# WE-Autopilot/red_gym

Hardware: AMD Instinct MI355X
Metric: env steps/sec (all envs), 1080-beam lidar (higher is better)
Workload: dtype f64; 1 GPU; 65536 envs x 1 agent(s) per GPU, example_map, 1080 beams, RK4 single-track, noise+iTTC, lap logic, autoreset; random actions; envs_per_gpu=65536, agents=1, num_beams=1080, map=example_map

## Files before the change

### include/f110_hip.h

```cpp
#ifndef F110_HIP_H
#define F110_HIP_H

#include <stdint.h>

#ifdef __cplusplus
extern "C" {
#endif

#define F110_OK 0
#define F110_E_INVALID (-1)
#define F110_E_HIP (-2)
#define F110_E_NOMAP (-3)
#define F110_E_INDEX (-4)
#define F110_E_UNBOUND (-5)

#define F110_MAX_CARS (1 << 26)
#define F110_MAX_AGENTS 32
#define F110_MAX_MAPS 4096
#define F110_MAX_NOISE_SLOTS 64
#define F110_NOISE_INITIAL_ROWS 1024
#define F110_NUM_PARAMS 18
#define F110_RK4 1
#define F110_EULER 2

// ... 86 lines not shown
int f110_noise_set_floor(f110_handle *h, int64_t lo, void *stream);
int f110_noise_info(f110_handle *h, int64_t *lo, int64_t *hi, int64_t *cap, int32_t *slots, int64_t *bytes);
int f110_noise_read(f110_handle *h, int32_t slot, int64_t row0, int64_t n_rows, double *out_host);

#define F110_DEVERR_NOISE_WINDOW 0x1u
#define F110_DEVERR_BOUNDS 0x2u
#define F110_DEVERR_QP_LIMIT 0x4u
int f110_device_errors(f110_handle *h, uint32_t *flags_out);

int f110_bind(f110_handle *h, const f110_buffers *bufs);

int f110_reset(f110_handle *h, const double *poses_dev, const uint8_t *mask_dev, void *stream);

int f110_step(f110_handle *h, const double *actions_dev, void *stream);

int64_t f110_pack_env_size(f110_handle *h);
int f110_pack_env(f110_handle *h, int32_t env, double *out_dev, void *stream);

int f110_set_scan_stages(f110_handle *h, const char *spec);

int f110_set_scan_order(f110_handle *h, const int32_t *order_dev);
int f110_launch_epoch(f110_handle *h, int64_t *epoch);

#define F110_GRAPH_NODES 0
#define F110_GRAPH_CAPTURE 1
typedef struct f110_graph f110_graph;
int f110_graph_create(f110_handle *h, const double *actions_dev, int32_t how, f110_graph **out);
int f110_graph_launch(f110_graph *g, void *stream);
int f110_graph_info(f110_graph *g, int32_t *nodes, const char *dot_path);
void f110_graph_destroy(f110_graph *g);

int f110_profile_begin(f110_handle *h, int32_t max_launches);
int f110_profile_every(f110_handle *h, int32_t every);
int f110_profile_end(f110_handle *h, double *scan_ms_total, int32_t *launches);

int f110_pure_pursuit_prepare(f110_handle *h, const double *waypoints, int32_t M, double cell, double margin, void *stream);
int f110_pure_pursuit(f110_handle *h, const double *waypoints, int32_t M, double lookahead, double vgain,
                      double wheelbase, double max_reacquire, const double *state, int32_t n,
                      double *actions, void *stream);

int64_t f110_pure_pursuit_workspace(int32_t total_points, int32_t K);
int f110_pure_pursuit_tracks(f110_handle *h, const double *waypoints, const int32_t *offsets_dev,
                             const int32_t *offsets_host, int32_t K, const int32_t *track_of_car, double lookahead,
                             double vgain, double wheelbase, double max_reacquire, const double *state, int32_t n,
                             double *actions, double *workspace, int32_t boxes_valid, void *stream);

// ... 363 lines not shown
```

### red_gym_amd/_lib.py

```python
import ctypes as C
import os

_HERE = os.path.dirname(os.path.abspath(__file__))
LIB_PATH = os.environ.get('F110_LIB') or os.path.join(_HERE, 'libf110_hip.so')

F110_MAX_AGENTS = 32
F110_MAX_NOISE_SLOTS = 64
F110_MAX_MAPS = 4096
F110_NUM_PARAMS = 18
F110_RK4, F110_EULER = 1, 2
E_INVALID, E_HIP, E_NOMAP, E_INDEX, E_UNBOUND = -1, -2, -3, -4, -5

PARAM_KEYS = ['mu', 'C_Sf', 'C_Sr', 'lf', 'lr', 'h', 'm', 'I', 's_min', 's_max', 'sv_min', 'sv_max',
              'v_switch', 'a_max', 'v_min', 'v_max', 'width', 'length']


class Config(C.Structure):
    _fields_ = [('num_envs', C.c_int32), ('num_agents', C.c_int32), ('num_beams', C.c_int32),
                ('theta_dis', C.c_int32), ('integrator', C.c_int32), ('ego_idx', C.c_int32),
                ('device', C.c_int32), ('autoreset', C.c_int32), ('fov', C.c_double), ('eps', C.c_double),
                ('max_range', C.c_double), ('timestep', C.c_double), ('ttc_thresh', C.c_double),
                ('params', C.c_double * F110_NUM_PARAMS)]


# ... 196 lines not shown
    'f110_set_params_slots': [_VP, _VP, _I32],
    'f110_set_params_slot': [_VP, _I32, _VP, _I32],
    'f110_assign_params': [_VP, _VP],
    'f110_set_side_distance_slots': [_VP, _VP, _I32],
    'f110_set_noise_table': [_VP, _VP, _I64],
    'f110_set_noise_slot': [_VP, _I32, _VP, _I64],
    'f110_set_noise_generator': [_VP, _I32, _VP, _D],
    'f110_assign_noise': [_VP, _VP],
    'f110_set_noise_per_env': [_VP, _VP, _D],
    'f110_noise_ensure': [_VP, _I64, _VP],
    'f110_noise_prefetch': [_VP, _I64],
    'f110_noise_set_floor': [_VP, _I64, _VP],
    'f110_noise_info': [_VP, C.POINTER(C.c_int64), C.POINTER(C.c_int64), C.POINTER(C.c_int64), C.POINTER(C.c_int32), C.POINTER(C.c_int64)],
    'f110_noise_read': [_VP, _I32, _I64, _I64, _VP],
    'f110_device_errors': [_VP, C.POINTER(C.c_uint32)],
    'f110_bind': [_VP, C.POINTER(Buffers)],
    'f110_reset': [_VP, _VP, _VP, _VP],
    'f110_step': [_VP, _VP, _VP],
    'f110_pack_env_size': [_VP],
    'f110_pack_env': [_VP, _I32, _VP, _VP],
    'f110_set_scan_stages': [_VP, C.c_char_p],
    'f110_launch_epoch': [_VP, C.POINTER(C.c_int64)],
    'f110_set_scan_order': [_VP, _VP],
    'f110_graph_create': [_VP, _VP, _I32, C.POINTER(_VP)],
    'f110_graph_launch': [_VP, _VP],
    'f110_graph_info': [_VP, C.POINTER(C.c_int32), C.c_char_p],
    'f110_graph_destroy': [_VP],
    'f110_pure_pursuit': [_VP, _VP, _I32, _D, _D, _D, _D, _VP, _I32, _VP, _VP],
    'f110_pure_pursuit_prepare': [_VP, _VP, _I32, _D, _D, _VP],
    'f110_pure_pursuit_workspace': [_I32, _I32],
    'f110_pure_pursuit_tracks': [_VP, _VP, _VP, _VP, _I32, _VP, _D, _D, _D, _D, _VP, _I32, _VP, _VP, _I32, _VP],
    'f110_progress_validate': [_VP, _VP, _I32, _VP, _VP, _VP, _VP, _VP, _I32],
    'f110_progress_install': [_VP, _VP, _VP, _I32, _VP, _VP, _VP, _VP, _VP, _I32],
    'f110_progress_bind': [_VP, C.POINTER(ProgressBuffers)],
    'f110_progress_update': [_VP, _VP],
    'f110_shaping_validate': [C.POINTER(ShapingConfig), _I32],
    'f110_shaping_install': [_VP, C.POINTER(ShapingConfig)],
    'f110_shaping_bind': [_VP, C.POINTER(ShapingBuffers)],
    'f110_shaping_update': [_VP, _VP],
    'f110_shaping_terms': [C.POINTER(ShapingConfig), _VP, _VP, _VP, _I32, _VP, _VP, _VP, _VP, _VP, _VP],
    'f110_shaping_terms_bits': [C.POINTER(ShapingConfig), _VP, _VP, _VP, _I32, _VP, _VP, _VP, _VP, _VP, _VP],
    'f110_pathfollow_validate': [C.POINTER(PathFollowConfig), _I32],
    'f110_pathfollow_install': [_VP, C.POINTER(PathFollowConfig)],
    'f110_pathfollow_bind': [_VP, C.POINTER(PathFollowBuffers)],
    'f110_pathfollow_act': [_VP, _VP, _VP, _VP],
    'f110_pathfollow_update': [_VP, _VP],
# ... 135 lines not shown
```

### red_gym_amd/csrc/f110_handle.h

```cpp
#pragma once
#include "f110_common.h"
#include "f110_device.h"
#include "f110_map.h"
#include "f110_noise.h"
#include "f110_plangrid.h"
#include "f110_scan_plan.h"

namespace f110 { struct OppPair; }

struct PlanGridDev {
    PlanGrid g;
    DevBuf<uint8_t> d_count; DevBuf<uint16_t> d_cand;
    hipError_t upload(const PlanGrid &geometry, const std::vector<uint8_t> &count, const std::vector<uint16_t> &cand)
    {
        hipError_t e = d_count.upload(count.data(), count.size());
        if (e == hipSuccess) e = d_cand.upload(cand.data(), cand.size());
        g = geometry; g.count = d_count.get(); g.cand = d_cand.get();
        return e;
    }
};

struct NoiseRows {
    const double *base;
    int cap, mask, slots;
// ... 83 lines not shown
    struct Replay {
        bool on = false, bound = false;
        f110_replay_config cfg;
        int rows = 0, cols = 0;
        f110_replay_buffers bufs;
    } replay;
    struct Episodes {
        bool on = false, bound = false;
        f110_episodes_config cfg;
        f110_episodes_buffers bufs;
    } episodes;
    const int32_t *scan_order = nullptr;
    DevBuf<uint32_t> d_err;
    std::vector<double> h_side;
    DevBuf<double> d_side_slots;
    int side_n_slots = 0;
    std::vector<double> h_side_slot0;
    double side_slots_max = 0.0;
    struct MapSlot {
        DevBuf<uint16_t> d_cells, d_cells_far;
        DevBuf<double> d_lut, d_lut_lds, d_dt;
        MapDev dev;
        bool used = false, ident = false, pow2 = false;
    };
    MapSlot slots[F110_MAX_MAPS];
    DevBuf<MapDev> d_maps;
    DevBuf<int32_t> d_env_map;
    std::vector<int32_t> h_env_map;
    bool multi = false;
    bool wg_single = false;
    bool ident = false, pow2 = false;
    double theta_inc = 0;
    std::vector<Event> prof_ev;
    int prof_n = 0, prof_every = 1, prof_seq = 0;
    bool prof_on = false;
};

int check_device(const f110_handle *h, const char *who);
int noise_init(f110_handle *h);
int alloc_opp_pairs(f110_handle *h);
```

### red_gym_amd/csrc/f110_map.h

```cpp
#pragma once
#include <hip/hip_runtime.h>
#include <stddef.h>
#include <stdint.h>

#pragma clang fp contract(off)

namespace f110 {

constexpr int LUT_LDS = 1024;
constexpr unsigned SLOT_OOB = 0, SLOT_FAR = LUT_LDS - 1;
constexpr unsigned LDS_RANKS = LUT_LDS - 2;
constexpr unsigned OFF_FAR = 8 * SLOT_FAR;
constexpr unsigned CODE_ESC = 65535;
__host__ __device__ inline unsigned cell_code(unsigned rank) { return rank < LDS_RANKS ? 8u * (rank + 1u) : OFF_FAR; }
__host__ __device__ inline int map_rows_padded(int H) { return ((H + 2 + 7) >> 3) << 3; }
__host__ __device__ inline size_t map_cells(int H, int W) { return (size_t)((W >> 3) + 2) * map_rows_padded(H) * 8; }
__host__ __device__ inline size_t cell_elem(int r, int c, int Hp) { return ((size_t)((c >> 3) + 1) * Hp + (size_t)(r + 1)) * 8 + (size_t)(c & 7); }

struct MapDev {
    const uint16_t *cells;
    const uint16_t *cells_far;
    unsigned cells_bytes;
    unsigned strip_bytes;
    const double *lut;
    const double *lut_lds;
    const double *dt;
    int H, W;
    double res, rinv, ox, oy, oc, os, wres, hres, oob;
    unsigned lut_len;
};

}
```

### red_gym_amd/csrc/f110_mapgen.h

```cpp
#pragma once
#include "f110_map.h"

#pragma clang fp contract(off)

namespace f110 {

constexpr unsigned EDT_NONE = 0xffffffffu;

static __global__ __launch_bounds__(256) void edt_columns_kernel(const uint8_t *mask, int H, int W, unsigned *g)
{
    const int x = blockIdx.x * blockDim.x + threadIdx.x;
    if (x >= W) return;
    unsigned d = EDT_NONE;
    for (int y = 0; y < H; y++) {
        const size_t i = (size_t)y * W + x;
        d = mask[i] ? (d == EDT_NONE ? EDT_NONE : d + 1) : 0u;
        g[i] = d;
    }
    d = EDT_NONE;
    for (int y = H - 1; y >= 0; y--) {
        const size_t i = (size_t)y * W + x;
        d = mask[i] ? (d == EDT_NONE ? EDT_NONE : d + 1) : 0u;
        const unsigned up = g[i];
        g[i] = d < up ? d : up;
// ... 107 lines not shown
    return word_prefix[v >> 5] + __popc(bits[v >> 5] & ((1u << (v & 31)) - 1u));
}

static __global__ __launch_bounds__(256) void map_encode_kernel(const unsigned *d2, int H, int W, int Hp, const unsigned *bits,
                                                         const unsigned *word_prefix, double res, uint16_t *cells,
                                                         uint16_t *cells_far, double *dt)
{
    const size_t i = (size_t)blockIdx.x * blockDim.x + threadIdx.x;
    if (i >= (size_t)H * W) return;
    const unsigned v = d2[i];
    const unsigned rank = d2_rank(bits, word_prefix, v);
    const size_t t = cell_elem((int)(i / W), (int)(i % W), Hp);
    cells[t] = (uint16_t)cell_code(rank);
    cells_far[t] = (uint16_t)(rank < CODE_ESC ? rank : CODE_ESC);
    dt[i] = res * sqrt((double)v);
}

static __global__ __launch_bounds__(256) void map_fill_border_kernel(uint16_t *cells, uint16_t *cells_far, size_t n)
{
    const size_t i = (size_t)blockIdx.x * blockDim.x + threadIdx.x;
    if (i >= n) return;
    cells[i] = 0;
    cells_far[i] = 0;
}

static __global__ __launch_bounds__(256) void map_lut_kernel(const unsigned *bits, int n_words, const unsigned *word_prefix, double res,
                                                      double *lut, unsigned n_lut)
{
    const int w = blockIdx.x * blockDim.x + threadIdx.x;
    if (w >= n_words) return;
    unsigned b = bits[w], rank = word_prefix[w];
    while (b && rank < n_lut) {
        const int bit = __ffs(b) - 1;
        b &= b - 1;
        lut[rank++] = res * sqrt((double)((unsigned)w * 32u + (unsigned)bit));
    }
}


struct TrackSeg { double ax, ay, ex, ey, inv_l2; };
constexpr int TRACK_CHUNK = 256;

static __global__ __launch_bounds__(256) void track_mask_kernel(const double *pts, int n_pts, int closed, int H, int W, double x0,
                                                         double y0, double pixel, double offset, double half_stroke,
                                                         uint8_t *mask)
{
// ... 33 lines not shown
```

### red_gym_amd/csrc/f110_maps.hip

```cpp
#include "f110_handle.h"
#include "f110_mapgen.h"

static int commit_map(f110_handle *h, int slot, f110_handle::MapSlot &&ns, int H, int W, double res, double ox, double oy, double oc,
                      double os, double oob)
{
    MapDev &m = ns.dev;
    memset(&m, 0, sizeof(m));
    m.cells = ns.d_cells.get(); m.cells_far = ns.d_cells_far.get(); m.lut = ns.d_lut.get(); m.lut_lds = ns.d_lut_lds.get(); m.dt = ns.d_dt.get();
    m.H = H; m.W = W; m.strip_bytes = (unsigned)map_rows_padded(H) * 16u; m.cells_bytes = (unsigned)(ns.d_cells.size() * sizeof(uint16_t));
    m.res = res; m.rinv = 1.0 / res;
    m.ox = ox; m.oy = oy; m.oc = oc; m.os = os;
    m.wres = W * res;
    m.hres = H * res;
    m.oob = oob;
    m.lut_len = (unsigned)ns.d_lut.size();
    int e = 0;
    ns.pow2 = std::frexp(res, &e) == 0.5;
    ns.ident = (oc == 1.0 && os == 0.0);
    ns.used = true;
    if (!h->d_maps.get()) {
        DevBuf<MapDev> maps;
        HIP_TRY(maps.alloc(F110_MAX_MAPS));
        HIP_TRY(hipMemset(maps.get(), 0, sizeof(MapDev) * F110_MAX_MAPS));
        h->d_maps = std::move(maps);
    }
    HIP_TRY(hipMemcpy(h->d_maps.get() + slot, &m, sizeof(MapDev), hipMemcpyHostToDevice));
    h->slots[slot] = std::move(ns);
    h->ident = h->pow2 = true;
    for (const auto &u : h->slots)
        if (u.used) { h->ident = h->ident && u.ident; h->pow2 = h->pow2 && u.pow2; }
// ... 255 lines not shown
```

### red_gym_amd/csrc/f110_scan.h

```cpp
#pragma once
#include "f110_bounds.h"
#include "f110_device.h"
#include "f110_map.h"
#include "f110_scan_plan.h"

#pragma clang fp contract(off)

namespace f110 {

constexpr int REFILL_MIN_IDLE = 44;

typedef unsigned u32x4 __attribute__((ext_vector_type(4)));
struct MapView {
    __amdgpu_buffer_rsrc_t cells_rsrc;
    u32x4 cells_words;
    unsigned row_bias, strip_m16;
    const MapDev *desc;
    int H, W;
    double res, rinv, ox, oy, oc, os, wres, hres;
    double nox, noy;
    F110_BOUNDS_ONLY(uint32_t *err = nullptr; unsigned cells_bytes = 0;)
    __device__ void init(const MapDev &m)
    {
        F110_BOUNDS_ONLY(cells_bytes = m.cells_bytes;)
        cells_rsrc = __builtin_amdgcn_make_buffer_rsrc(const_cast<uint16_t *>(m.cells), 0, (int)m.cells_bytes, 0x00020000);
        cells_words.x = __builtin_amdgcn_readfirstlane((unsigned)(unsigned long long)m.cells);
        cells_words.y = __builtin_amdgcn_readfirstlane((unsigned)((unsigned long long)m.cells >> 32) & 0xffffu);
        cells_words.z = __builtin_amdgcn_readfirstlane(m.cells_bytes); cells_words.w = __builtin_amdgcn_readfirstlane(0x00020000u);
        row_bias = m.strip_bytes + 16u; strip_m16 = m.strip_bytes - 16u; desc = &m; H = m.H; W = m.W; res = m.res; rinv = m.rinv;
        ox = m.ox; oy = m.oy; oc = m.oc; os = m.os; wres = m.wres; hres = m.hres;
        nox = -m.ox * m.rinv; noy = -m.oy * m.rinv;
    }
};

struct ScanDev {
    int nb, theta_dis;
    double fov, eps, max_range, inc;
    unsigned long long inc_fx;
    int cs_len;
    const double2 *cs;
};

template <bool IDENT, bool POW2>
__device__ inline void cell_index(const MapView &m, double x, double y, int &ci, int &ri)
{
    double xr = 0, yr = 0, qx, qy;
    if (IDENT && POW2) {
        qx = __builtin_fma(x, m.rinv, m.nox);
        qy = __builtin_fma(y, m.rinv, m.noy);
    } else {
// ... 18 lines not shown
    }
}

__device__ inline unsigned cell_offset(const MapView &m, int ci, int ri)
{
    const int cc = med3_i32(ci, -1, m.W);
    const int rr = med3_i32(ri, -1, m.H);
    unsigned row16;
    asm("v_lshl_add_u32 %0, %1, 4, %2" : "=v"(row16) : "v"(rr), "s"(m.row_bias));
    unsigned rc;
    asm("v_lshl_add_u32 %0, %1, 1, %2" : "=v"(rc) : "v"(cc), "v"(row16));
    return (unsigned)(__mul24(cc >> 3, (int)m.strip_m16) + (int)rc);
}

template <bool IDENT, bool POW2>
__device__ inline double dist_lookup(const MapView &m, const double *lds_lut, double x, double y)
{
    int ci, ri;
    cell_index<IDENT, POW2>(m, x, y, ci, ri);
    const unsigned off = cell_offset(m, ci, ri);
    unsigned code = (unsigned)(unsigned short)__builtin_amdgcn_raw_buffer_load_b16(m.cells_rsrc, (int)off, 0, 0);
#if defined(F110_BOUNDS)
    F110_BCHK(off + 2u <= m.cells_bytes, BT_LUT_CODE, m.err);
    F110_BCHK(code <= OFF_FAR && (code & 7u) == 0u, BT_LUT_CODE, m.err);
    code = code <= OFF_FAR ? (code & ~7u) : 0u;
#endif
    double d = *reinterpret_cast<const double *>(reinterpret_cast<const char *>(lds_lut) + code);
    asm volatile("" : "+v"(d));
    return d;
}

template <bool IDENT, bool POW2>
__device__ inline double dist_lookup_far(const MapView &m, double x, double y)
{
    int ci, ri;
    cell_index<IDENT, POW2>(m, x, y, ci, ri);
    unsigned off = cell_offset(m, ci, ri);
    const MapDev *dp = m.desc;
    asm volatile("" : "+s"(dp));
#if defined(F110_BOUNDS)
    F110_BCHK(off + 2u <= dp->cells_bytes, BT_CELLS_FAR, m.err);
    if (off + 2u > dp->cells_bytes) off = 0u;
#endif
    unsigned rank = *reinterpret_cast<const uint16_t *>(reinterpret_cast<const char *>(dp->cells_far) + (size_t)off);
    const bool inside = (unsigned)ri < (unsigned)m.H && (unsigned)ci < (unsigned)m.W;
#if defined(F110_BOUNDS)
    F110_BCHK(rank == CODE_ESC || rank < dp->lut_len, BT_LUT_RANK, m.err);
    if (rank != CODE_ESC && rank >= dp->lut_len) rank = 0u;
// ... 219 lines not shown
    double ttc_thresh;
    uint8_t *in_collision;
    const uint8_t *pending_reset;
    int reset_only;
    const uint16_t *chunk_beam0;
    const int32_t *order;
    int wg_single;
    int n_maps;
    const double *side_slots;
    const int32_t *env_params;
    int side_n_slots;
    float *out_f32;
    double *out_f64;
    uint32_t *lookups;
};

static_assert(__is_trivially_copyable(ScanArgs), "ScanArgs is copied into the kernarg segment byte for byte");
static_assert(offsetof(ScanArgs, maps) == 0, "kernarg re-read assumes the argument block starts with ScanArgs");
static_assert(sizeof(((ScanArgs *)0)->stage_cars) == SCAN_MAX_STAGES * sizeof(int) &&
              sizeof(((ScanArgs *)0)->stage_log2w) == SCAN_MAX_STAGES * sizeof(int), "stage list capacity");
static_assert(sizeof(ScanArgs) <= 4096, "kernarg segment size");

constexpr int SCAN_MIN_WAVES = 8;
template <bool IDENT, bool POW2, int SM>
__global__ __launch_bounds__(SCAN_THREADS, SCAN_MIN_WAVES) void scan_kernel(ScanArgs a)
{
    constexpr bool STEP = SM >= 1;
    __shared__ struct __attribute__((aligned(16))) { double lut[LUT_LDS]; int chunk0[MAX_CHUNKS]; } s_mem;
    double *const s_lut = s_mem.lut;
    int *const s_chunk0 = s_mem.chunk0;
#if defined(__HIP_DEVICE_COMPILE__)
    const ScanArgs *rare = (const ScanArgs *)__builtin_amdgcn_kernarg_segment_ptr();
#else
    const ScanArgs *rare = &a;
#endif
    const int nb = a.scan.nb;
    const int wave = __builtin_amdgcn_readfirstlane(threadIdx.x >> 6), lane = threadIdx.x & 63;
    const int wg_single = rare->wg_single;
    const int wid = wg_single ? (int)blockIdx.x : (int)blockIdx.x * SCAN_WAVES + wave;
    int wpc, car, part, lg;
    {
        int t = wid, c = 0, st = 0;
        const int ns = rare->n_stages;
        for (; st < ns; st++) {
            const int cars_s = rare->stage_cars[st], w = cars_s << rare->stage_log2w[st];
            if (t < w) break;
            t -= w; c += cars_s;
        }
        lg = st < ns ? rare->stage_log2w[st] : 0;
        wpc = 1 << lg; car = st < ns ? c + (t >> lg) : a.n_cars; part = t & (wpc - 1);
    }
    int car_c = rare->car_base + min(car, a.n_cars - 1);
    if (rare->order) car_c = rare->order[car_c];
    const int env_c = a.agents == 1 ? car_c : car_c / a.agents;
    F110_BCHK(rare->n_stages >= 1 && rare->n_stages <= SCAN_MAX_STAGES, BT_STAGE_LIST, rare->dev_err);
    int map_slot = a.env_map ? a.env_map[env_c] : 0;
#if defined(F110_BOUNDS)
    F110_BCHK((unsigned)map_slot < (unsigned)rare->n_maps, BT_MAP_SLOT, rare->dev_err);
    if ((unsigned)map_slot >= (unsigned)rare->n_maps) map_slot = 0;
#endif
    const MapDev &md = a.maps[map_slot];
    {
        const double2 *src = reinterpret_cast<const double2 *>(md.lut_lds);
        double2 *dst = reinterpret_cast<double2 *>(s_lut);
        for (int i = threadIdx.x; i < LUT_LDS / 2; i += SCAN_THREADS) dst[i] = src[i];
        if (SCAN_WAVES > 1 && wg_single)
            for (int k = 1; k < SCAN_WAVES; k++)
                for (int i = threadIdx.x + k * WAVE; i < LUT_LDS / 2; i += SCAN_THREADS) dst[i] = src[i];
    }
    static_assert(MAX_CHUNKS <= WAVE, "one pass of one wave stages the chunk table");
    if ((int)threadIdx.x < ((nb + 63) >> 6)) s_chunk0[threadIdx.x] = a.chunk_beam0[threadIdx.x];
    __syncthreads();
    MapView mv;
    mv.init(md);
    F110_BOUNDS_ONLY(mv.err = rare->dev_err;)
    if (car >= a.n_cars) return;
    car = car_c;
    const int nch = (nb + 63) >> 6;
    const int my_chunks = nch > part ? (nch - part + wpc - 1) >> lg : 0;
    const int owns_last = my_chunks > 0 && ((nch - 1) & (wpc - 1)) == part;
    const int nbl = my_chunks * 64 - (owns_last ? nch * 64 - nb : 0);
    if (a.reset_only && !a.pending_reset[env_c]) return;

    const double px = a.pose_src[(size_t)car * a.pose_stride];
    const double py = a.pose_src[(size_t)car * a.pose_stride + 1];
    const double yaw = a.pose_src[(size_t)car * a.pose_stride + a.yaw_off];
    const double eps = a.scan.eps, max_range = a.scan.max_range;

    const double vel = STEP ? a.state[(size_t)car * 7 + 3] : 0.0;
    const bool do_ttc = STEP && vel != 0.0;
    const double cand = a.ttc_thresh * fabs(vel) * 1.000000001;
    const double side_pre = do_ttc ? (rare->side_max + cand) + 1e-9 * (fabs(rare->side_max) + cand) : -__builtin_inf();
    const double *__restrict__ ns = nullptr;
    if (STEP) {
        const int row = a.noise_step[car];
        int slot = a.env_noise ? a.env_noise[env_c] : 0;
#if defined(F110_BOUNDS)
// ... 189 lines not shown
```

### red_gym_amd/csrc/f110_scan_plan.h

```cpp
#pragma once
#include "../../include/f110_hip.h"

#include <algorithm>
#include <cstdlib>
#include <cstring>
#include <vector>

int fail(int code, const char *fmt, ...);

namespace f110 {

constexpr int WAVE = 64;
constexpr int SCAN_WAVES = 2;
constexpr int SCAN_THREADS = SCAN_WAVES * WAVE;
constexpr int SCAN_MAX_STAGES = 8, SCAN_MAX_LOG2W = 3;
constexpr int MAX_CHUNKS = 64;

struct StageSpec { int cars, lg; };

inline bool parse_stage_spec(const char *p, std::vector<StageSpec> &spec, const char **why)
{
    spec.clear();
    int stars = 0;
    if (!p || !*p) { *why = "empty"; return false; }
    for (;;) {
        int cars = -1, lg = 0;
// ... 25 lines not shown
    std::vector<StageSpec> spec = override_spec;
    if (spec.empty()) {
        int wpc = n_cars <= 1024 ? 8 : (n_cars <= 2048 ? 4 : 1);
        const int nch = (num_beams + 63) / 64;
        while (wpc > 1 && wpc > nch) wpc /= 2;
        if (wpc > 1 || nch < 8) return {{n_cars, wpc >= 8 ? 3 : wpc >= 4 ? 2 : wpc >= 2 ? 1 : 0}};
        const int tail = std::min(agents >= 2 ? 4096 : 2048, n_cars / 2);
        spec = {{-1, 0}, {tail, 2}};
    }
    int fixed = 0;
    for (StageSpec &x : spec) if (x.cars >= 0) { x.cars -= x.cars % SCAN_WAVES; fixed += x.cars; }
    if (fixed > n_cars) { spec = {{-1, 0}}; fixed = 0; }
    bool star = false;
    for (StageSpec &x : spec) if (x.cars < 0 && !star) { x.cars = n_cars - fixed; star = true; }
    if (!star) spec.push_back({n_cars - fixed, 0});
    std::vector<StageSpec> stv;
    for (const StageSpec &x : spec) if (x.cars > 0) stv.push_back(x);
    for (size_t i = 0; i + 1 < stv.size(); i++)
        if (stv[i].cars % SCAN_WAVES) return {{n_cars, 0}};
    if (stv.size() > (size_t)SCAN_MAX_STAGES) return {{n_cars, 0}};
    return stv;
}

struct ScanPlanIn {
    int n_cars, agents, num_beams;
    const std::vector<StageSpec> *stages;
    bool step;
    const char *stores;
    bool multi, wg_single;
    int kind;
};

struct ScanLaunch {
    int car_base, n_cars;
    int kind;
    int sm;
    int n_stages, stage_cars[SCAN_MAX_STAGES], stage_log2w[SCAN_MAX_STAGES];
    int grid, block;
    bool wg_single, order, events;
};

template <typename EnvKind>
int plan_scan(const ScanPlanIn &in, EnvKind env_kind, std::vector<ScanLaunch> &out)
{
    const bool split = in.multi && in.kind != 3;
    const int num_envs = in.n_cars / in.agents;
    out.clear();
    for (int e0 = 0, e1 = num_envs; e0 < num_envs; e0 = e1) {
        ScanLaunch l = {};
        l.kind = split ? env_kind(e0) : in.kind;
        if (split)
            for (e1 = e0 + 1; e1 < num_envs && env_kind(e1) == l.kind; e1++) {}
        l.car_base = e0 * in.agents; l.n_cars = (e1 - e0) * in.agents;
        l.wg_single = in.multi && in.wg_single; l.order = in.step && !in.multi; l.events = in.step && e0 == 0;
        const std::vector<StageSpec> stv = scan_stage_list(*in.stages, l.n_cars, in.agents, in.num_beams);
        if (stv.size() < 1 || stv.size() > (size_t)SCAN_MAX_STAGES) return fail(F110_E_INVALID, "scan launch: %d stages (1..%d)", (int)stv.size(), SCAN_MAX_STAGES);
        long long cars = 0, waves = 0;
        for (const StageSpec &x : stv) {
            if (x.cars < 0 || x.lg < 0 || x.lg > SCAN_MAX_LOG2W) return fail(F110_E_INVALID, "scan launch: stage (%d cars, 2^%d waves per car) out of range", x.cars, x.lg);
            if (in.multi && !l.wg_single && (l.car_base + cars) % SCAN_WAVES) return fail(F110_E_INVALID, "scan launch: a stage of two-wave workgroups on a map per env starts at car %lld", l.car_base + cars);
            l.stage_cars[l.n_stages] = x.cars; l.stage_log2w[l.n_stages++] = x.lg;
            cars += x.cars; waves += x.cars << x.lg;
        }
        if (cars != l.n_cars) return fail(F110_E_INVALID, "scan launch: the stages cover %lld cars, the launch has %d", cars, l.n_cars);
        const bool plain = in.stores ? strcmp(in.stores, "plain") == 0 : l.n_cars > 327680;
        l.sm = !in.step ? 0 : plain ? 2 : 1;
        l.grid = (int)(l.wg_single ? waves : (waves + SCAN_WAVES - 1) / SCAN_WAVES);
        l.block = l.wg_single ? WAVE : SCAN_THREADS;
        out.push_back(l);
    }
    return F110_OK;
}

}
```

### red_gym_amd/csrc/f110_step.hip

```cpp
#include "f110_handle.h"
#include "f110_scan.h"
#include "f110_env.h"
#include "f110_mirrors.h"
#include "f110_noise_kernels.h"

int alloc_opp_pairs(f110_handle *h)
{
    if (h->cfg.num_agents < 2) return F110_OK;
    const size_t n = (size_t)h->cfg.num_envs * h->cfg.num_agents * (h->cfg.num_agents - 1);
    DevBuf<OppPair> pairs;
    DevBuf<uint8_t> was_pending;
    HIP_TRY(pairs.alloc(n));
    HIP_TRY(hipMemset(pairs.get(), 0, n * sizeof(OppPair)));
    HIP_TRY(was_pending.alloc((size_t)h->cfg.num_envs));
    HIP_TRY(hipMemset(was_pending.get(), 0, (size_t)h->cfg.num_envs));
    h->d_opp_pairs = std::move(pairs);
    h->d_was_pending = std::move(was_pending);
    return F110_OK;
}

struct KernelLaunch {
    const void *func;
    dim3 grid, block;
    unsigned shmem;
// ... 30 lines not shown
    memset(&s, 0, sizeof(s));
    ScanDev &d = s.scan;
    d.nb = h->cfg.num_beams; d.theta_dis = h->cfg.theta_dis; d.fov = h->cfg.fov; d.eps = h->cfg.eps;
    d.max_range = h->cfg.max_range; d.inc = h->theta_inc; d.inc_fx = (unsigned long long)std::llround(h->theta_inc * 1099511627776.0); d.cs_len = (int)h->d_cs.size(); d.cs = h->d_cs.get();
    s.maps = h->d_maps.get(); s.n_maps = F110_MAX_MAPS; s.n_cars = n_cars; s.agents = agents; s.chunk_beam0 = h->d_chunk0.get();
    s.pose_src = pose_src; s.pose_stride = pose_stride; s.yaw_off = yaw_off; s.out_f32 = out_f32; s.out_f64 = out_f64; s.lookups = lookups;
    return s;
}

static int check_scan_args(const ScanArgs &a, const char *who)
{
    if (a.n_cars < 1 || a.agents < 1 || a.scan.nb < 2 || a.scan.nb > MAX_CHUNKS * 64) return fail(F110_E_INVALID, "%s: %d cars, %d agents, %d beams", who, a.n_cars, a.agents, a.scan.nb);
    if (!a.maps || !a.scan.cs || a.scan.cs_len < a.scan.theta_dis || !a.chunk_beam0 || !a.pose_src) return fail(F110_E_INVALID, "%s: a table of the scan is missing (maps / {cos,sin} LUT / chunk order / poses)", who);
    if (!a.out_f32 && !a.out_f64) return fail(F110_E_INVALID, "%s: no output buffer", who);
    if (a.state && (!a.noise_step || !a.noise_base || a.noise_cap < 1 || !a.beam_cosines || !a.in_collision || !a.pending_reset))
        return fail(F110_E_INVALID, "%s: a buffer of the step's scan is missing (noise / beam cosines / in_collision / pending_reset)", who);
    if (!a.state && a.reset_only) return fail(F110_E_INVALID, "%s: reset_only without the step's buffers", who);
    return F110_OK;
}

#define SCAN_KERNELS(SM) {(const void *)&scan_kernel<false, false, SM>, (const void *)&scan_kernel<true, false, SM>, \
                          (const void *)&scan_kernel<false, true, SM>, (const void *)&scan_kernel<true, true, SM>}
static const void *const scan_kernels[3][4] = {SCAN_KERNELS(0), SCAN_KERNELS(1), SCAN_KERNELS(2)};

static int run_scan(const f110_handle *h, const ScanArgs &a, const Sink &k, hipEvent_t ev0 = nullptr, hipEvent_t ev1 = nullptr)
{
    if (int rc = check_scan_args(a, "scan launch")) return rc;
    static const char *stores_env = getenv("F110_SCAN_STORES");
    ScanPlanIn in;
    in.n_cars = a.n_cars; in.agents = a.agents; in.num_beams = a.scan.nb; in.stages = &h->stages; in.step = a.state != nullptr;
    in.stores = stores_env; in.multi = a.env_map != nullptr; in.wg_single = h->wg_single; in.kind = h->ident | h->pow2 << 1;
    std::vector<ScanLaunch> plan;
    if (int rc = plan_scan(in, [h](int env) { const f110_handle::MapSlot &m = h->slots[h->h_env_map[env]]; return m.ident | m.pow2 << 1; }, plan))
        return rc;
    for (const ScanLaunch &l : plan) {
        ScanArgs s = a;
        s.car_base = l.car_base; s.n_cars = l.n_cars; s.wg_single = l.wg_single; s.order = l.order ? h->scan_order : nullptr;
        s.n_stages = l.n_stages; memcpy(s.stage_cars, l.stage_cars, sizeof(s.stage_cars)); memcpy(s.stage_log2w, l.stage_log2w, sizeof(s.stage_log2w));
        if (int rc = emit(k, scan_kernels[l.sm][l.kind], dim3(l.grid), dim3(l.block), 0, s, l.events ? ev0 : nullptr,
                          l.events ? ev1 : nullptr))
            return rc;
    }
    return F110_OK;
}

static int run_step(f110_handle *h, const double *actions, int reset_only, const Sink &st)
{
    const f110_config &c = h->cfg;
    const f110_buffers &b = h->bufs;
    const int N = c.num_envs * c.num_agents;
    const bool prof = h->prof_on && !st.record && (h->prof_seq++ % h->prof_every) == h->prof_every / 2 && (size_t)(2 * h->prof_n + 1) < h->prof_ev.size();
    hipEvent_t ev0 = prof ? h->prof_ev[2 * h->prof_n].get() : nullptr, ev1 = prof ? h->prof_ev[2 * h->prof_n + 1].get() : nullptr;
    int rc;

    if (h->noise.per_env) {
        NoiseGenArgs g;
        memset(&g, 0, sizeof(g));
        g.gen = h->noise.d_env_gen.get(); g.seeds = h->noise.d_env_seed.get(); g.base = h->noise.d_env_rows.get(); g.mask = 0; g.cap = 1; g.nb = c.num_beams;
        g.pcg_tab = h->noise.d_pcg_tab.get(); g.env_row = b.noise_step; g.env_row_stride = c.num_agents; g.n_env = c.num_envs;
        g.reset_only = reset_only; g.env_pending = b.pending_reset;
        if ((rc = emit(st, (const void *)&noise_rows_kernel, dim3((c.num_envs + 3) / 4), dim3(256), 0, g))) return rc;
    }
// ... 398 lines not shown
```

### red_gym_amd/engine.py

```python
import contextlib
import ctypes as C
import os

import numpy as np
import torch

from . import _lib
from .base_classes import integrator_code
from .maps import load_map
from .progress import ProgressTracker
from .shaping import RewardShaper
from .pathfollow import PathFollower
from .replay import ReplayBuffer
from .episodes import EpisodeTracker

DEFAULT_PARAMS = {'mu': 1.0489, 'C_Sf': 4.718, 'C_Sr': 5.4562, 'lf': 0.15875, 'lr': 0.17145, 'h': 0.074,
                  'm': 3.74, 'I': 0.04712, 's_min': -0.4189, 's_max': 0.4189, 'sv_min': -3.2, 'sv_max': 3.2,
                  'v_switch': 7.319, 'a_max': 9.51, 'v_min': -5.0, 'v_max': 20.0, 'width': 0.31, 'length': 0.58}

_TORCH_DTYPES = {
    'state': torch.float64, 'steer_buf': torch.float64, 'steer_cnt': torch.int32, 'noise_step': torch.int32,
    'spawn': torch.float64, 'start_rot': torch.float64, 'near_start': torch.uint8, 'toggles': torch.int32,
    'current_time': torch.float64, 'pending_reset': torch.uint8, 'scans': torch.float32,
    'scans_f64': torch.float64, 'pose_snap': torch.float64, 'collisions': torch.uint8,
# ... 373 lines not shown
        _lib.check(self.lib.f110_get_map_slot_dt(self._h, int(slot), _np_ptr(out)))
        return out

    def update_params(self, params, agent_idx=-1):
        pv = params_vec(params)
        _lib.check(self.lib.f110_update_params(self._h, _np_ptr(pv), int(agent_idx)))
        if agent_idx < 0:
            self.params = dict(params)

    @on_own_device
    def reset(self, poses, mask=None):
        if tuple(poses.shape) != (self.B, self.A, 3):
            raise ValueError('Number of poses for reset does not match number of agents.')
        poses = poses.to(device=self.device, dtype=torch.float64).contiguous()
        if mask is not None:
            mask = mask.to(device=self.device, dtype=torch.uint8).contiguous()
            self._steps_exact = False
        else:
            self.host_steps_bound = 0
            self._steps_exact = not self.autoreset
        if self._noise_floor > 0:
            self._set_noise_floor(0)
        self.ready_noise(may_raise_floor=False)
        _lib.check(self.lib.f110_reset(self._h, _ptr(poses), _ptr(mask), self._stream()))
        self.host_steps_bound += 1
        self._keep = (poses, mask)

    @on_own_device
    def step(self, actions):
        if tuple(actions.shape) != (self.B, self.A, 2):
            raise ValueError('actions must have shape (%d, %d, 2)' % (self.B, self.A))
        if actions.dtype != torch.float64 or not actions.is_contiguous() or actions.device != self.device:
            actions = actions.to(device=self.device, dtype=torch.float64).contiguous()
        self.ready_noise()
        _lib.check(self.lib.f110_step(self._h, _ptr(actions), self._stream()))
        if not self._in_capture:
            self.host_steps_bound += 1
        self._keep = actions

    @contextlib.contextmanager
    def capturing(self):
        self._in_capture = True
        try:
            yield
        finally:
            self._in_capture = False
# ... 162 lines not shown
                                                     _ptr(tracks.workspace), int(tracks.boxes_valid), self._stream()))
        tracks.boxes_valid = True
        self._keep_tracks = (tracks, track_of_car)
        return out.view(self.B, self.A, 2) if state is None else out

    @on_own_device
    def pack_env(self, env=0):
        if getattr(self, '_pack_dev', None) is None:
            n = int(self.lib.f110_pack_env_size(self._h))
            self._pack_dev = torch.empty((n,), dtype=torch.float64, device=self.device)
            self._pack_host = torch.empty((n,), dtype=torch.float64).pin_memory()
        _lib.check(self.lib.f110_pack_env(self._h, int(env), _ptr(self._pack_dev), self._stream()))
        self._pack_host.copy_(self._pack_dev, non_blocking=True)
        torch.cuda.current_stream(self.device).synchronize()
        return self._pack_host.numpy()

    def set_scan_stages(self, spec=None):
        _lib.check(self.lib.f110_set_scan_stages(self._h, None if spec is None else spec.encode()))

    def launch_epoch(self):
        e = C.c_int64(0)
        _lib.check(self.lib.f110_launch_epoch(self._h, C.byref(e)))
        return e.value

    def profile_begin(self, max_launches, every=1):
        _lib.check(self.lib.f110_profile_every(self._h, int(every)))
        _lib.check(self.lib.f110_profile_begin(self._h, int(max_launches)))

    def profile_end(self):
        ms, n = C.c_double(0), C.c_int32(0)
        _lib.check(self.lib.f110_profile_end(self._h, C.byref(ms), C.byref(n)))
        return ms.value, n.value

    def close(self):
        if getattr(self, '_h', None) is not None and self._h:
            self.tracker.close()
            self.shaper.close()
            self.follower.close()
            self.replay.close()
            self.episodes.close()
            torch.cuda.synchronize(self.device)
            flags = self.device_errors() if os.environ.get('F110_CHECK_DEVICE_ERRORS') == '1' else 0
            self.lib.f110_destroy(self._h)
            self._h = None
            if flags:
                raise RuntimeError('f110 device error word 0x%x at close (bit 0: noise row outside the table, bit 1: an index '
# ... 56 lines not shown
```

Before: 107.8 million env-steps/s.

## Add compact-LUT scan kernel variants chosen by reachable-cell far-share analysis

Builds 256- and 512-entry compacted cell-code tables and LDS LUT images for the primary map. Cells whose rank exceeds the compact size are redirected to the far path. At reset, a host flood fill from the spawn poses estimates how often reachable cells would hit the far path, and a compact scan kernel is selected when that share is small. This is meant to shrink the per-block LDS footprint and staging cost of the lidar kernel. In exchange it adds extra device memory, a one-time host sync and copy at reset, and more far-path lookups for rare cells.

```diff
diff --git a/include/f110_hip.h b/include/f110_hip.h
--- a/include/f110_hip.h
+++ b/include/f110_hip.h
@@ -132,6 +132,9 @@
 int f110_set_scan_order(f110_handle *h, const int32_t *order_dev);
 int f110_launch_epoch(f110_handle *h, int64_t *epoch);
 
+int f110_scan_form_learn(f110_handle *h, const double *poses_dev, void *stream);
+int f110_scan_form_info(f110_handle *h, int32_t n_cars, int32_t *form, double *out_share);
+
 #define F110_GRAPH_NODES 0
 #define F110_GRAPH_CAPTURE 1
 typedef struct f110_graph f110_graph;
diff --git a/red_gym_amd/_lib.py b/red_gym_amd/_lib.py
--- a/red_gym_amd/_lib.py
+++ b/red_gym_amd/_lib.py
@@ -242,6 +242,8 @@
     'f110_set_scan_stages': [_VP, C.c_char_p],
     'f110_launch_epoch': [_VP, C.POINTER(C.c_int64)],
     'f110_set_scan_order': [_VP, _VP],
+    'f110_scan_form_info': [_VP, _I32, C.POINTER(C.c_int32), C.POINTER(C.c_double)],
+    'f110_scan_form_learn': [_VP, _VP, _VP],
     'f110_graph_create': [_VP, _VP, _I32, C.POINTER(_VP)],
     'f110_graph_launch': [_VP, _VP],
     'f110_graph_info': [_VP, C.POINTER(C.c_int32), C.c_char_p],
diff --git a/red_gym_amd/csrc/f110_handle.h b/red_gym_amd/csrc/f110_handle.h
--- a/red_gym_amd/csrc/f110_handle.h
+++ b/red_gym_amd/csrc/f110_handle.h
@@ -129,6 +129,12 @@
         DevBuf<double> d_lut, d_lut_lds, d_dt;
         MapDev dev;
         bool used = false, ident = false, pow2 = false;
+        DevBuf<uint16_t> d_cells_c[N_COMPACT];
+        DevBuf<double> d_lut_lds_c[N_COMPACT];
+        bool compact = false;
+        double compact_out[N_COMPACT] = {1.0, 1.0};
+        bool reach_known = false;
+        double reach_out[N_COMPACT] = {1.0, 1.0};
     };
     MapSlot slots[F110_MAX_MAPS];
     DevBuf<MapDev> d_maps;
diff --git a/red_gym_amd/csrc/f110_map.h b/red_gym_amd/csrc/f110_map.h
--- a/red_gym_amd/csrc/f110_map.h
+++ b/red_gym_amd/csrc/f110_map.h
@@ -13,6 +13,12 @@
 constexpr unsigned OFF_FAR = 8 * SLOT_FAR;
 constexpr unsigned CODE_ESC = 65535;
 __host__ __device__ inline unsigned cell_code(unsigned rank) { return rank < LDS_RANKS ? 8u * (rank + 1u) : OFF_FAR; }
+constexpr int N_COMPACT = 2;
+constexpr int LUT_COMPACT[N_COMPACT] = {256, 512};
+__host__ __device__ constexpr unsigned compact_off_far(int S) { return 8u * (unsigned)(S - 1); }
+__host__ __device__ constexpr unsigned compact_code(unsigned code, int S) { return code < compact_off_far(S) ? code : compact_off_far(S); }
+__host__ __device__ constexpr int compact_index(int S) { return S == 256 ? 0 : S == 512 ? 1 : -1; }
+static_assert(compact_index(LUT_COMPACT[0]) == 0 && compact_index(LUT_COMPACT[1]) == 1, "compact_index names LUT_COMPACT's entries");
 __host__ __device__ inline int map_rows_padded(int H) { return ((H + 2 + 7) >> 3) << 3; }
 __host__ __device__ inline size_t map_cells(int H, int W) { return (size_t)((W >> 3) + 2) * map_rows_padded(H) * 8; }
 __host__ __device__ inline size_t cell_elem(int r, int c, int Hp) { return ((size_t)((c >> 3) + 1) * Hp + (size_t)(r + 1)) * 8 + (size_t)(c & 7); }
@@ -28,6 +34,8 @@
     int H, W;
     double res, rinv, ox, oy, oc, os, wres, hres, oob;
     unsigned lut_len;
+    const uint16_t *cells_c[N_COMPACT];
+    const double *lut_lds_c[N_COMPACT];
 };
 
 }
diff --git a/red_gym_amd/csrc/f110_mapgen.h b/red_gym_amd/csrc/f110_mapgen.h
--- a/red_gym_amd/csrc/f110_mapgen.h
+++ b/red_gym_amd/csrc/f110_mapgen.h
@@ -153,6 +153,27 @@
     if (i >= n) return;
     cells[i] = 0;
     cells_far[i] = 0;
+}
+
+static __global__ __launch_bounds__(256) void map_compact_kernel(const uint16_t *cells, size_t n, uint16_t *out0, uint16_t *out1,
+                                                                 unsigned *counts)
+{
+    __shared__ unsigned s_cnt[1 + N_COMPACT];
+    if (threadIdx.x < 1 + N_COMPACT) s_cnt[threadIdx.x] = 0;
+    __syncthreads();
+    const size_t i = (size_t)blockIdx.x * blockDim.x + threadIdx.x;
+    if (i < n) {
+        const unsigned code = cells[i];
+        out0[i] = (uint16_t)compact_code(code, LUT_COMPACT[0]);
+        out1[i] = (uint16_t)compact_code(code, LUT_COMPACT[1]);
+        if (code > cell_code(0)) {
+            atomicAdd(&s_cnt[0], 1u);
+            if (code >= compact_off_far(LUT_COMPACT[0])) atomicAdd(&s_cnt[1], 1u);
+            if (code >= compact_off_far(LUT_COMPACT[1])) atomicAdd(&s_cnt[2], 1u);
+        }
+    }
+    __syncthreads();
+    if (threadIdx.x < 1 + N_COMPACT && s_cnt[threadIdx.x]) atomicAdd(&counts[threadIdx.x], s_cnt[threadIdx.x]);
 }
 
 static __global__ __launch_bounds__(256) void map_lut_kernel(const unsigned *bits, int n_words, const unsigned *word_prefix, double res,
diff --git a/red_gym_amd/csrc/f110_maps.hip b/red_gym_amd/csrc/f110_maps.hip
--- a/red_gym_amd/csrc/f110_maps.hip
+++ b/red_gym_amd/csrc/f110_maps.hip
@@ -1,11 +1,44 @@
 #include "f110_handle.h"
 #include "f110_mapgen.h"
 
+constexpr size_t COMPACT_MAX_BYTES = (size_t)64 << 20;
+static void build_compact(f110_handle::MapSlot &ns)
+{
+    const size_t n = ns.d_cells.size();
+    if (n * sizeof(uint16_t) > COMPACT_MAX_BYTES) return;
+    DevBuf<uint16_t> cells[N_COMPACT];
+    DevBuf<double> img[N_COMPACT];
+    DevBuf<unsigned> counts;
+    double classic[LUT_COMPACT[N_COMPACT - 1]];
+    unsigned cnt[1 + N_COMPACT] = {};
+    bool ok = counts.alloc(1 + N_COMPACT) == hipSuccess && hipMemset(counts.get(), 0, sizeof(cnt)) == hipSuccess &&
+              hipMemcpy(classic, ns.d_lut_lds.get(), sizeof(classic), hipMemcpyDeviceToHost) == hipSuccess;
+    for (int i = 0; ok && i < N_COMPACT; i++) {
+        std::vector<double> v(classic, classic + LUT_COMPACT[i]);
+        v.back() = -0.0;
+        ok = cells[i].alloc(n) == hipSuccess && img[i].upload(v.data(), v.size()) == hipSuccess;
+    }
+    if (ok) {
+        hipLaunchKernelGGL(map_compact_kernel, dim3((unsigned)((n + 255) / 256)), dim3(256), 0, nullptr, ns.d_cells.get(), n,
+                           cells[0].get(), cells[1].get(), counts.get());
+        ok = hipGetLastError() == hipSuccess && hipMemcpy(cnt, counts.get(), sizeof(cnt), hipMemcpyDeviceToHost) == hipSuccess;
+    }
+    if (!ok) { (void)hipGetLastError(); return; }
+    for (int i = 0; i < N_COMPACT; i++) {
+        ns.d_cells_c[i] = std::move(cells[i]);
+        ns.d_lut_lds_c[i] = std::move(img[i]);
+        ns.compact_out[i] = cnt[0] ? (double)cnt[1 + i] / (double)cnt[0] : 0.0;
+    }
+    ns.compact = true;
+}
+
 static int commit_map(f110_handle *h, int slot, f110_handle::MapSlot &&ns, int H, int W, double res, double ox, double oy, double oc,
                       double os, double oob)
 {
+    if (slot == 0) build_compact(ns);
     MapDev &m = ns.dev;
     memset(&m, 0, sizeof(m));
+    for (int i = 0; i < N_COMPACT; i++) { m.cells_c[i] = ns.d_cells_c[i].get(); m.lut_lds_c[i] = ns.d_lut_lds_c[i].get(); }
     m.cells = ns.d_cells.get(); m.cells_far = ns.d_cells_far.get(); m.lut = ns.d_lut.get(); m.lut_lds = ns.d_lut_lds.get(); m.dt = ns.d_dt.get();
     m.H = H; m.W = W; m.strip_bytes = (unsigned)map_rows_padded(H) * 16u; m.cells_bytes = (unsigned)(ns.d_cells.size() * sizeof(uint16_t));
     m.res = res; m.rinv = 1.0 / res;
diff --git a/red_gym_amd/csrc/f110_scan.h b/red_gym_amd/csrc/f110_scan.h
--- a/red_gym_amd/csrc/f110_scan.h
+++ b/red_gym_amd/csrc/f110_scan.h
@@ -19,13 +19,14 @@
     int H, W;
     double res, rinv, ox, oy, oc, os, wres, hres;
     double nox, noy;
-    F110_BOUNDS_ONLY(uint32_t *err = nullptr; unsigned cells_bytes = 0;)
-    __device__ void init(const MapDev &m)
+    F110_BOUNDS_ONLY(uint32_t *err = nullptr; unsigned cells_bytes = 0; unsigned off_far = OFF_FAR;)
+    __device__ void init(const MapDev &m, const uint16_t *cells, unsigned far_code)
     {
-        F110_BOUNDS_ONLY(cells_bytes = m.cells_bytes;)
-        cells_rsrc = __builtin_amdgcn_make_buffer_rsrc(const_cast<uint16_t *>(m.cells), 0, (int)m.cells_bytes, 0x00020000);
-        cells_words.x = __builtin_amdgcn_readfirstlane((unsigned)(unsigned long long)m.cells);
-        cells_words.y = __builtin_amdgcn_readfirstlane((unsigned)((unsigned long long)m.cells >> 32) & 0xffffu);
+        F110_BOUNDS_ONLY(cells_bytes = m.cells_bytes; off_far = far_code;)
+        (void)far_code;
+        cells_rsrc = __builtin_amdgcn_make_buffer_rsrc(const_cast<uint16_t *>(cells), 0, (int)m.cells_bytes, 0x00020000);
+        cells_words.x = __builtin_amdgcn_readfirstlane((unsigned)(unsigned long long)cells);
+        cells_words.y = __builtin_amdgcn_readfirstlane((unsigned)((unsigned long long)cells >> 32) & 0xffffu);
         cells_words.z = __builtin_amdgcn_readfirstlane(m.cells_bytes); cells_words.w = __builtin_amdgcn_readfirstlane(0x00020000u);
         row_bias = m.strip_bytes + 16u; strip_m16 = m.strip_bytes - 16u; desc = &m; H = m.H; W = m.W; res = m.res; rinv = m.rinv;
         ox = m.ox; oy = m.oy; oc = m.oc; os = m.os; wres = m.wres; hres = m.hres;
@@ -90,8 +91,8 @@
     unsigned code = (unsigned)(unsigned short)__builtin_amdgcn_raw_buffer_load_b16(m.cells_rsrc, (int)off, 0, 0);
 #if defined(F110_BOUNDS)
     F110_BCHK(off + 2u <= m.cells_bytes, BT_LUT_CODE, m.err);
-    F110_BCHK(code <= OFF_FAR && (code & 7u) == 0u, BT_LUT_CODE, m.err);
-    code = code <= OFF_FAR ? (code & ~7u) : 0u;
+    F110_BCHK(code <= m.off_far && (code & 7u) == 0u, BT_LUT_CODE, m.err);
+    code = code <= m.off_far ? (code & ~7u) : 0u;
 #endif
     double d = *reinterpret_cast<const double *>(reinterpret_cast<const char *>(lds_lut) + code);
     asm volatile("" : "+v"(d));
@@ -357,11 +358,15 @@
 static_assert(sizeof(ScanArgs) <= 4096, "kernarg segment size");
 
 constexpr int SCAN_MIN_WAVES = 8;
-template <bool IDENT, bool POW2, int SM>
+static_assert(N_COMPACT == SCAN_COMPACT_N && LUT_COMPACT[0] == SCAN_COMPACT_S[0] && LUT_COMPACT[1] == SCAN_COMPACT_S[1],
+              "the plan's compact sizes are the map tables'");
+template <bool IDENT, bool POW2, int SM, int LUTN = LUT_LDS>
 __global__ __launch_bounds__(SCAN_THREADS, SCAN_MIN_WAVES) void scan_kernel(ScanArgs a)
 {
     constexpr bool STEP = SM >= 1;
-    __shared__ struct __attribute__((aligned(16))) { double lut[LUT_LDS]; int chunk0[MAX_CHUNKS]; } s_mem;
+    constexpr bool COMPACT = LUTN != LUT_LDS;
+    static_assert(!COMPACT || (compact_index(LUTN) >= 0 && STEP && IDENT && POW2), "compact forms: the step's scan, kind 3");
+    __shared__ struct __attribute__((aligned(16))) { double lut[LUTN]; int chunk0[MAX_CHUNKS]; } s_mem;
     double *const s_lut = s_mem.lut;
     int *const s_chunk0 = s_mem.chunk0;
 #if defined(__HIP_DEVICE_COMPILE__)
@@ -371,7 +376,7 @@
 #endif
     const int nb = a.scan.nb;
     const int wave = __builtin_amdgcn_readfirstlane(threadIdx.x >> 6), lane = threadIdx.x & 63;
-    const int wg_single = rare->wg_single;
+    const int wg_single = COMPACT ? 1 : rare->wg_single;
     const int wid = wg_single ? (int)blockIdx.x : (int)blockIdx.x * SCAN_WAVES + wave;
     int wpc, car, part, lg;
     {
@@ -396,18 +401,19 @@
 #endif
     const MapDev &md = a.maps[map_slot];
     {
-        const double2 *src = reinterpret_cast<const double2 *>(md.lut_lds);
+        const double2 *src = reinterpret_cast<const double2 *>(COMPACT ? md.lut_lds_c[compact_index(LUTN) & 1] : md.lut_lds);
         double2 *dst = reinterpret_cast<double2 *>(s_lut);
-        for (int i = threadIdx.x; i < LUT_LDS / 2; i += SCAN_THREADS) dst[i] = src[i];
+        for (int i = threadIdx.x; i < LUTN / 2; i += SCAN_THREADS) dst[i] = src[i];
         if (SCAN_WAVES > 1 && wg_single)
             for (int k = 1; k < SCAN_WAVES; k++)
-                for (int i = threadIdx.x + k * WAVE; i < LUT_LDS / 2; i += SCAN_THREADS) dst[i] = src[i];
+                for (int i = threadIdx.x + k * WAVE; i < LUTN / 2; i += SCAN_THREADS) dst[i] = src[i];
     }
     static_assert(MAX_CHUNKS <= WAVE, "one pass of one wave stages the chunk table");
     if ((int)threadIdx.x < ((nb + 63) >> 6)) s_chunk0[threadIdx.x] = a.chunk_beam0[threadIdx.x];
     __syncthreads();
     MapView mv;
-    mv.init(md);
+    if (COMPACT) mv.init(md, md.cells_c[compact_index(LUTN) & 1], compact_off_far(LUTN));
+    else mv.init(md, md.cells, OFF_FAR);
     F110_BOUNDS_ONLY(mv.err = rare->dev_err;)
     if (car >= a.n_cars) return;
     car = car_c;
diff --git a/red_gym_amd/csrc/f110_scan_plan.h b/red_gym_amd/csrc/f110_scan_plan.h
--- a/red_gym_amd/csrc/f110_scan_plan.h
+++ b/red_gym_amd/csrc/f110_scan_plan.h
@@ -2,6 +2,7 @@
 #include "../../include/f110_hip.h"
 
 #include <algorithm>
+#include <cmath>
 #include <cstdlib>
 #include <cstring>
 #include <vector>
@@ -73,6 +74,69 @@
     return stv;
 }
 
+constexpr int SCAN_COMPACT_N = 2;
+constexpr int SCAN_COMPACT_S[SCAN_COMPACT_N] = {256, 512};
+constexpr double SCAN_COMPACT_CAP = 0.004;
+constexpr int SCAN_COMPACT_MIN_CARS = 32768;
+
+inline int scan_compact_choice(const double *out_share, int n_cars, int agents, double cap = SCAN_COMPACT_CAP,
+                               int min_cars = SCAN_COMPACT_MIN_CARS)
+{
+    if (n_cars < min_cars || agents != 1) return 0;
+    for (int i = 0; i < SCAN_COMPACT_N; i++)
+        if (out_share[i] < cap) return SCAN_COMPACT_S[i];
+    return 0;
+}
+
+template <typename CodeAt>
+void scan_reach_shares(int H, int W, CodeAt code_at, unsigned code_zero, const unsigned *off_far, const double *poses,
+                       int pose_stride, int n_cars, double ox, double oy, double rinv, double *share)
+{
+    std::vector<int> label((size_t)H * W, 0);
+    std::vector<double> comp_share;
+    std::vector<int> stack;
+    double sum[SCAN_COMPACT_N] = {};
+    for (int i = 0; i < n_cars; i++) {
+        const double qx = std::floor((poses[(size_t)i * pose_stride] - ox) * rinv), qy = std::floor((poses[(size_t)i * pose_stride + 1] - oy) * rinv);
+        if (!(qx >= 0 && qx < W && qy >= 0 && qy < H)) continue;
+        const int r0 = (int)qy, c0 = (int)qx;
+        if (!(code_at(r0, c0) > code_zero)) continue;
+        int &l0 = label[(size_t)r0 * W + c0];
+        if (!l0) {
+            const int id = (int)(comp_share.size() / SCAN_COMPACT_N) + 1;
+            size_t n_free = 0, n_out[SCAN_COMPACT_N] = {};
+            l0 = id;
+            stack.push_back(r0 * W + c0);
+            while (!stack.empty()) {
+                const int at = stack.back(), r = at / W, c = at % W;
+                stack.pop_back();
+                const unsigned code = code_at(r, c);
+                n_free++;
+                for (int k = 0; k < SCAN_COMPACT_N; k++) n_out[k] += code >= off_far[k];
+                for (int dr = -1; dr <= 1; dr++)
+                    for (int dc = -1; dc <= 1; dc++) {
+                        const int rr = r + dr, cc = c + dc;
+                        if (rr < 0 || rr >= H || cc < 0 || cc >= W || label[(size_t)rr * W + cc] || !(code_at(rr, cc) > code_zero)) continue;
+                        label[(size_t)rr * W + cc] = id;
+                        stack.push_back(rr * W + cc);
+                    }
+            }
+            for (int k = 0; k < SCAN_COMPACT_N; k++) comp_share.push_back((double)n_out[k] / (double)n_free);
+        }
+        for (int k = 0; k < SCAN_COMPACT_N; k++) sum[k] += comp_share[(size_t)(label[(size_t)r0 * W + c0] - 1) * SCAN_COMPACT_N + k];
+    }
+    for (int k = 0; k < SCAN_COMPACT_N; k++) share[k] = n_cars > 0 ? sum[k] / (double)n_cars : 1.0;
+}
+
+inline int scan_form_override(const char *v)
+{
+    if (!v) return -1;
+    if (!strcmp(v, "classic")) return 0;
+    if (!strcmp(v, "compact256")) return 256;
+    if (!strcmp(v, "compact512")) return 512;
+    return -1;
+}
+
 struct ScanPlanIn {
     int n_cars, agents, num_beams;
     const std::vector<StageSpec> *stages;
@@ -80,6 +144,7 @@
     const char *stores;
     bool multi, wg_single;
     int kind;
+    int compact = 0;
 };
 
 struct ScanLaunch {
@@ -89,6 +154,7 @@
     int n_stages, stage_cars[SCAN_MAX_STAGES], stage_log2w[SCAN_MAX_STAGES];
     int grid, block;
     bool wg_single, order, events;
+    int lut;
 };
 
 template <typename EnvKind>
@@ -103,7 +169,8 @@
         if (split)
             for (e1 = e0 + 1; e1 < num_envs && env_kind(e1) == l.kind; e1++) {}
         l.car_base = e0 * in.agents; l.n_cars = (e1 - e0) * in.agents;
-        l.wg_single = in.multi && in.wg_single; l.order = in.step && !in.multi; l.events = in.step && e0 == 0;
+        l.lut = in.step && !in.multi && in.kind == 3 ? in.compact : 0;
+        l.wg_single = (in.multi && in.wg_single) || l.lut != 0; l.order = in.step && !in.multi; l.events = in.step && e0 == 0;
         const std::vector<StageSpec> stv = scan_stage_list(*in.stages, l.n_cars, in.agents, in.num_beams);
         if (stv.size() < 1 || stv.size() > (size_t)SCAN_MAX_STAGES) return fail(F110_E_INVALID, "scan launch: %d stages (1..%d)", (int)stv.size(), SCAN_MAX_STAGES);
         long long cars = 0, waves = 0;
diff --git a/red_gym_amd/csrc/f110_step.hip b/red_gym_amd/csrc/f110_step.hip
--- a/red_gym_amd/csrc/f110_step.hip
+++ b/red_gym_amd/csrc/f110_step.hip
@@ -76,6 +76,66 @@
 #define SCAN_KERNELS(SM) {(const void *)&scan_kernel<false, false, SM>, (const void *)&scan_kernel<true, false, SM>, \
                           (const void *)&scan_kernel<false, true, SM>, (const void *)&scan_kernel<true, true, SM>}
 static const void *const scan_kernels[3][4] = {SCAN_KERNELS(0), SCAN_KERNELS(1), SCAN_KERNELS(2)};
+static const void *const scan_kernels_compact[N_COMPACT][2] = {
+    {(const void *)&scan_kernel<true, true, 1, LUT_COMPACT[0]>, (const void *)&scan_kernel<true, true, 2, LUT_COMPACT[0]>},
+    {(const void *)&scan_kernel<true, true, 1, LUT_COMPACT[1]>, (const void *)&scan_kernel<true, true, 2, LUT_COMPACT[1]>}};
+
+static int scan_form_forced() { static const int forced = scan_form_override(getenv("F110_SCAN_FORM")); return forced; }
+static int scan_form(const f110_handle *h, int n_cars)
+{
+    const int forced = scan_form_forced();
+    const f110_handle::MapSlot &m = h->slots[0];
+    if (!m.compact || h->multi || !(h->ident && h->pow2)) return 0;
+    if (forced >= 0) return forced;
+    return m.reach_known ? scan_compact_choice(m.reach_out, n_cars, h->cfg.num_agents) : 0;
+}
+
+extern "C" int f110_scan_form_learn(f110_handle *h, const double *poses_dev, void *stream)
+{
+    if (!h || !poses_dev) return fail(F110_E_INVALID, "f110_scan_form_learn: null argument");
+    if (!h->has_map) return fail(F110_E_NOMAP, "Map is not set for scan simulator.");
+    f110_handle::MapSlot &m = h->slots[0];
+    const int N = h->cfg.num_envs * h->cfg.num_agents;
+    const double none[N_COMPACT] = {};
+    if (!m.compact || m.reach_known || h->multi || !(h->ident && h->pow2) || scan_form_forced() >= 0 ||
+        scan_compact_choice(none, N, h->cfg.num_agents) == 0)
+        return F110_OK;
+    if (int rc = check_device(h, "f110_scan_form_learn")) return rc;
+    hipStream_t st = (hipStream_t)stream;
+    hipStreamCaptureStatus cap = hipStreamCaptureStatusNone;
+    if (hipStreamIsCapturing(st, &cap) != hipSuccess) { (void)hipGetLastError(); return F110_OK; }
+    if (cap != hipStreamCaptureStatusNone) return F110_OK;
+    try {
+        std::vector<double> poses((size_t)N * 3);
+        std::vector<uint16_t> cells(m.d_cells.size());
+        HIP_TRY(hipStreamSynchronize(st));
+        HIP_TRY(hipMemcpy(poses.data(), poses_dev, poses.size() * sizeof(double), hipMemcpyDeviceToHost));
+        HIP_TRY(hipMemcpy(cells.data(), m.d_cells.get(), cells.size() * sizeof(uint16_t), hipMemcpyDeviceToHost));
+        const MapDev &d = m.dev;
+        const int Hp = map_rows_padded(d.H);
+        const unsigned off_far[N_COMPACT] = {compact_off_far(LUT_COMPACT[0]), compact_off_far(LUT_COMPACT[1])};
+        scan_reach_shares(d.H, d.W, [&](int r, int c) { return (unsigned)cells[cell_elem(r, c, Hp)]; }, cell_code(0), off_far,
+                          poses.data(), 3, N, d.ox, d.oy, d.rinv, m.reach_out);
+    } catch (const std::bad_alloc &) {
+        return F110_OK;
+    }
+    m.reach_known = true;
+    h->epoch++;
+    return F110_OK;
+}
+
+extern "C" int f110_scan_form_info(f110_handle *h, int32_t n_cars, int32_t *form, double *out_share)
+{
+    if (!h || !form || !out_share || n_cars < 1) return fail(F110_E_INVALID, "f110_scan_form_info: bad arguments");
+    if (!h->has_map) return fail(F110_E_NOMAP, "Map is not set for scan simulator.");
+    const f110_handle::MapSlot &m = h->slots[0];
+    *form = scan_form(h, n_cars);
+    for (int i = 0; i < N_COMPACT; i++) {
+        out_share[i] = m.compact ? m.compact_out[i] : 1.0;
+        out_share[N_COMPACT + i] = m.reach_known ? m.reach_out[i] : -1.0;
+    }
+    return F110_OK;
+}
 
 static int run_scan(const f110_handle *h, const ScanArgs &a, const Sink &k, hipEvent_t ev0 = nullptr, hipEvent_t ev1 = nullptr)
 {
@@ -84,6 +144,7 @@
     ScanPlanIn in;
     in.n_cars = a.n_cars; in.agents = a.agents; in.num_beams = a.scan.nb; in.stages = &h->stages; in.step = a.state != nullptr;
     in.stores = stores_env; in.multi = a.env_map != nullptr; in.wg_single = h->wg_single; in.kind = h->ident | h->pow2 << 1;
+    in.compact = in.step && !in.multi ? scan_form(h, a.n_cars) : 0;
     std::vector<ScanLaunch> plan;
     if (int rc = plan_scan(in, [h](int env) { const f110_handle::MapSlot &m = h->slots[h->h_env_map[env]]; return m.ident | m.pow2 << 1; }, plan))
         return rc;
@@ -91,7 +152,15 @@
         ScanArgs s = a;
         s.car_base = l.car_base; s.n_cars = l.n_cars; s.wg_single = l.wg_single; s.order = l.order ? h->scan_order : nullptr;
         s.n_stages = l.n_stages; memcpy(s.stage_cars, l.stage_cars, sizeof(s.stage_cars)); memcpy(s.stage_log2w, l.stage_log2w, sizeof(s.stage_log2w));
-        if (int rc = emit(k, scan_kernels[l.sm][l.kind], dim3(l.grid), dim3(l.block), 0, s, l.events ? ev0 : nullptr,
+        const void *func = scan_kernels[l.sm][l.kind];
+        if (l.lut) {
+            const int ci = compact_index(l.lut);
+            const MapDev &m = h->slots[0].dev;
+            if (ci < 0 || l.sm < 1 || l.kind != 3 || !m.cells_c[ci] || !m.lut_lds_c[ci])
+                return fail(F110_E_INVALID, "scan launch: compact form %d without its tables (kind %d, sm %d)", l.lut, l.kind, l.sm);
+            func = scan_kernels_compact[ci][l.sm - 1];
+        }
+        if (int rc = emit(k, func, dim3(l.grid), dim3(l.block), 0, s, l.events ? ev0 : nullptr,
                           l.events ? ev1 : nullptr))
             return rc;
     }
diff --git a/red_gym_amd/engine.py b/red_gym_amd/engine.py
--- a/red_gym_amd/engine.py
+++ b/red_gym_amd/engine.py
@@ -419,6 +419,8 @@
         if self._noise_floor > 0:
             self._set_noise_floor(0)
         self.ready_noise(may_raise_floor=False)
+        if mask is None and not self._in_capture:
+            _lib.check(self.lib.f110_scan_form_learn(self._h, _ptr(poses), self._stream()))
         _lib.check(self.lib.f110_reset(self._h, _ptr(poses), _ptr(mask), self._stream()))
         self.host_steps_bound += 1
         self._keep = (poses, mask)
@@ -627,6 +629,12 @@
         e = C.c_int64(0)
         _lib.check(self.lib.f110_launch_epoch(self._h, C.byref(e)))
         return e.value
+
+    def scan_form(self, n_cars=None):
+        form, share = C.c_int32(0), (C.c_double * 4)()
+        n = self.N if n_cars is None else int(n_cars)
+        _lib.check(self.lib.f110_scan_form_info(self._h, n, C.byref(form), share))
+        return form.value, tuple(share)
 
     def profile_begin(self, max_launches, every=1):
         _lib.check(self.lib.f110_profile_every(self._h, int(every)))
```

New measurement: 111.2 million env-steps/s, median of 6. 3.1% higher.
